# tensorflow/compression

Measured on AMD Instinct MI355X. Metric: Mpixels/s encode+decode round-trip (bit-exact), higher is better.
Workload: dtype int32

## Files before the change

compression_amd/csrc/range_pipe.h:

```cpp
#pragma once

#ifndef TFC_PIPE_TIMING
#define TFC_PIPE_TIMING 0
#endif

namespace tfc {

constexpr int kPipeTile = 256;
constexpr int kPipeEscMax = 32;
constexpr unsigned int kPipeBlock = 16;
constexpr unsigned int kPipeNoCall = 0x0001FFFFu;
constexpr unsigned int kPipeAggregate = 1u << 30;
constexpr unsigned int kPipePrefix = 2u << 30;
constexpr unsigned int kPipeRowsMask = (1u << 30) - 1u;

struct PipeEncArgs {
  const uint16_t* fast16;
  const int2* rows_fast;
  int ntab;
  int tab_entries;
  unsigned int* calls;
  unsigned int* status;
  unsigned int* done;
  unsigned int* fallback;
// ... 560 lines not shown
#endif
    while ((((v = sync[L::kSeq + b % L::kSlots]) & ~(L::kLast | L::kBail)) != b + 1u) && !(v & L::kBail)) __builtin_amdgcn_s_sleep(1);
    asm volatile("" ::: "memory");
#if TFC_PIPE_TIMING
    waited_words += clock64() - c0;
#endif
    return v;
  };

  unsigned int wa[kPipeBlock], wb[kPipeBlock];
  unsigned int seq = wait_words(0u);
  bool bail = (seq & L::kBail) != 0u;
  if (!bail) read_words(wa, 0u, 0u);
  unsigned int dig_done = 0u;
  for (unsigned int b = 0; !bail; ++b) {
    const bool last = (seq & L::kLast) != 0u;
    read_words(wb, b % L::kSlots, 1u);
    const unsigned int seq_early = last ? 0u : sync[L::kSeq + (b + 1u) % L::kSlots];
    if (dig_done + L::kDigSlots <= b) {
#if TFC_PIPE_TIMING
      const unsigned long long c0 = clock64();
#endif
      while ((dig_done = sync[L::kDigDone]) + L::kDigSlots <= b) __builtin_amdgcn_s_sleep(1);
#if TFC_PIPE_TIMING
      waited_digits += clock64() - c0;
#endif
    }
    const unsigned int dslot = b % L::kDigSlots;
    dstage = area + L::kDig + dslot * L::kDigSlot + L::kDigStride * lane;
    ds_off = area_off + L::kDig + dslot * L::kDigSlot + L::kDigStride * lane;
    n = 0u;
    block(wa);
    if (lane == 0u) sync[L::kConsumed] = b + 1u;
    if (!last) {
      seq = ((seq_early & ~(L::kLast | L::kBail)) == b + 2u || (seq_early & L::kBail)) ? seq_early : wait_words(b + 1u);
      if (seq & L::kBail) { bail = true; break; }
      read_words(wa, (b + 1u) % L::kSlots, 0u);
    }
    block(wb);
    reinterpret_cast<uint2*>(area + L::kRec)[dslot * 64u + lane] = make_uint2(wpos, n);
    overflow |= (n != 0u && wpos + ((n + 15u) & ~15u) > pa.cap) ? 1u : 0u;
    wpos += n;
    asm volatile("s_waitcnt lgkmcnt(0)" ::: "memory");
    if (lane == 0u) sync[L::kDigPub] = b + 1u;
    if (__any(too_long)) {
      bail = true;
      if (lane == 0u) atomicOr(&pa.fallback[job], 1u);
      break;
    }
    if (last) break;
  }
  asm volatile("s_waitcnt lgkmcnt(0)" ::: "memory");
  if (lane == 0u) sync[L::kExit] = 1u;
  if (gi == 0u && lane == 0u) {
    g_pipe_clock[0] = clock64() - clk0;
    g_pipe_clock[1] = wall_clock64() - wall0;
    g_pipe_clock[4] = waited_words;
    g_pipe_clock[6] = waited_digits;
#if TFC_PIPE_TIMING
    g_enc_clock[0] = t_blocks; g_enc_clock[1] = n_blocks; g_enc_clock[2] = n_redone; g_enc_clock[3] = t_redo;
#endif
  }
  if (bail) return;
  if (live) {
    pa.stage_state[static_cast<size_t>(gi) * 64 + lane] = make_uint4(base, s1, (hd & 0xFFFFu) | (had << 31), rn);
    pa.stage_out[static_cast<size_t>(gi) * 64 + lane] = make_uint2(wpos, overflow);
  }
}

__global__ void __launch_bounds__(64) enc_chain_direct_kernel(const PipeChainJobs jobs, const PipeEncArgs pa) {
  constexpr unsigned int kRows = PipeEncChainLds::kRows;
  constexpr unsigned int kDigits = 2 * kRows;
  constexpr int kStride = lane_stride(kDigits + 8);
  __shared__ __attribute__((aligned(16))) unsigned char stage[64 * kStride];
  const unsigned int gi = blockIdx.x;
  const unsigned int job = gi / static_cast<unsigned int>(pa.groups_per_job);
  const unsigned int gidx = gi % static_cast<unsigned int>(pa.groups_per_job);
  if (__hip_atomic_load(&pa.fallback[job], __ATOMIC_RELAXED, __HIP_MEMORY_SCOPE_AGENT) != 0u) return;
  const PipeChainJob& J = jobs.job[job];
  const unsigned int lane = threadIdx.x;
  const int64_t s = static_cast<int64_t>(gidx) * 64 + lane;
  const bool live = s < jobs.streams;

  uint4 st = live ? J.state[s] : make_uint4(0u, 0xFFFFFFFFu, 0u, 0u);
  unsigned int base = st.x, s1 = st.y, hd = st.z & 0xFFFFu, had = st.z >> 31, rn = st.w;
  lanes_pin(base, s1, hd, rn);

  const unsigned int ds_off = static_cast<unsigned int>(reinterpret_cast<size_t>(
                                  (__attribute__((address_space(3))) unsigned char*)stage)) + kStride * lane;
  unsigned char* const dstage = stage + kStride * lane;
  unsigned char* const out = J.chunk + (live ? s : 0) * static_cast<int64_t>(pa.cap);
  unsigned int wpos = 0u, n = 0u, overflow = 0u;

  auto put = [&](unsigned int d, bool on) {
    *reinterpret_cast<unsigned short*>(dstage + n) = __builtin_bswap16(static_cast<unsigned short>(d));
    n += on ? 2u : 0u;
  };
  auto flush = [&]() {
#pragma unroll
    for (unsigned int c = 0; c < kDigits / 16u; ++c) {
      if (16u * c < n) {
        uint2 v[2];
        v[0] = reinterpret_cast<const uint2*>(dstage)[2 * c];
        v[1] = reinterpret_cast<const uint2*>(dstage)[2 * c + 1];
        if (wpos + 16u * c + 16u <= pa.cap) lanes_gstore16(out + wpos + 16u * c, v[0], v[1]);
        else overflow = 1u;
      }
    }
    wpos += n;
    n = 0u;
  };
  auto put_run = [&](unsigned int fill, unsigned int bytes) {
    flush();
    for (unsigned int k = 0; k < bytes; k += 2u) {
      const unsigned short be = static_cast<unsigned short>(fill);
      if (wpos + 2u <= pa.cap) lanes_gstore_elem(reinterpret_cast<unsigned short*>(out + wpos), be);
      else overflow = 1u;
      wpos += 2u;
    }
  };
  auto call = [&](unsigned int lo, unsigned int hi, bool act) __attribute__((always_inline)) {
    const unsigned int a = scale16(s1, lo);
    const unsigned int b = scale16(s1, hi) - 1u;
    const unsigned int bs = base + a;
    const unsigned int t1 = b - a;
    const bool carry = act && bs < a;
    const bool ren = act && (t1 >> 16) == 0u;
    const unsigned int e = bs >> 16;
    const bool solid = ren && e != 0xFFFFu;
    const bool ffff = ren && e == 0xFFFFu;
    const bool held = had != 0u;
    const unsigned int X = (hd + (carry ? 1u : 0u)) & 0xFFFFu;
    const bool emit = held && (solid || (carry && (!ffff || rn != 0u)));
    put(X, emit);
    const unsigned int run_out = !held ? 0u : solid ? rn : (carry && rn != 0u) ? (ffff ? rn - 1u : rn) : 0u;
    if (__any(run_out != 0u)) {
      if (run_out != 0u) put_run(carry ? 0u : 0xFFFFu, 2u * run_out);
    }
    if (solid) {
      hd = e; had = 1u; rn = 0u;
    } else if (ffff) {
      if (!held) { hd = 0xFFFFu; had = 1u; rn = 0u; }
      else if (!carry) { rn += 1u; }
      else if (rn == 0u) { hd = X; rn = 1u; }
      else { hd = 0u; rn = 1u; }
    } else if (carry && held) {
      had = 0u; rn = 0u;
    }
    base = act ? (ren ? bs << 16 : bs) : base;
    s1 = act ? (ren ? (t1 << 16) | 0xFFFFu : t1) : s1;
  };

  const unsigned int nt = static_cast<unsigned int>(pa.nt);
  const unsigned int* const status = pa.status + static_cast<size_t>(gi) * nt * 64 + lane;
  const unsigned int* const done = pa.done + static_cast<size_t>(gi) * nt;
  unsigned int avail = 0u;
  unsigned int tn = 0u;
  bool bail = false;
  auto ensure = [&](unsigned int need) {
    while (tn < nt && __any(live && avail < need)) {
      const unsigned int* const flag = done + tn;
      long long t0 = 0;
      bool timing = false;
      while (__hip_atomic_load(flag, __ATOMIC_RELAXED, __HIP_MEMORY_SCOPE_AGENT) == 0u) {
        const long long now = static_cast<long long>(wall_clock64());
        if (!timing) { t0 = now; timing = true; }
        else if (now - t0 > pa.poll_ticks) { bail = true; return; }
        __builtin_amdgcn_s_sleep(8);
      }
      __builtin_amdgcn_fence(__ATOMIC_ACQUIRE, "agent");
      avail = __hip_atomic_load(status + static_cast<size_t>(tn) * 64, __ATOMIC_RELAXED, __HIP_MEMORY_SCOPE_AGENT) & kPipeRowsMask;
      ++tn;
      if (__hip_atomic_load(&pa.fallback[job], __ATOMIC_RELAXED, __HIP_MEMORY_SCOPE_AGENT) != 0u) { bail = true; return; }
    }
  };

  const unsigned char* const mine = reinterpret_cast<const unsigned char*>(pa.calls + static_cast<size_t>(gi) * 64 * pa.rows) + 128u * lane;
  unsigned int w[kRows] = {}, wn[kRows] = {};
  auto load_rows = [&](unsigned int b) {
    const unsigned char* p = mine + static_cast<size_t>(b) * (64u * kRows * 4u);
#pragma unroll
    for (unsigned int c = 0; c < kRows / 4u; ++c) {
      const uint4 v = lanes_gload16(p + 16u * c);
      wn[4 * c] = v.x; wn[4 * c + 1] = v.y; wn[4 * c + 2] = v.z; wn[4 * c + 3] = v.w;
    }
  };
  auto block = [&](unsigned int w0, unsigned int w1, unsigned int w2, unsigned int w3, unsigned int w4, unsigned int w5,
                   unsigned int w6, unsigned int w7, unsigned int w8, unsigned int w9, unsigned int w10, unsigned int w11,
                   unsigned int w12, unsigned int w13, unsigned int w14, unsigned int w15) __attribute__((always_inline)) {
    const unsigned int base0 = base, s10 = s1, hd0 = hd, had0 = had;
    unsigned int flag = rn, na = ds_off + n;
    asm volatile(
        "s_mov_b64 s[56:57], exec\n\t"
        "v_mov_b32 v101, 0\n\tv_mov_b32 v103, 0\n\t"
        TFC_PENC_STEP(W0) TFC_PENC_STEP(W1) TFC_PENC_STEP(W2) TFC_PENC_STEP(W3)
        TFC_PENC_STEP(W4) TFC_PENC_STEP(W5) TFC_PENC_STEP(W6) TFC_PENC_STEP(W7)
        TFC_PENC_STEP(W8) TFC_PENC_STEP(W9) TFC_PENC_STEP(W10) TFC_PENC_STEP(W11)
        TFC_PENC_STEP(W12) TFC_PENC_STEP(W13) TFC_PENC_STEP(W14) TFC_PENC_STEP(W15)
        "s_mov_b64 exec, s[56:57]\n\t"
        "s_waitcnt lgkmcnt(0)\n\t"
        : [BASE] "+v"(base), [S] "+v"(s1), [H] "+v"(hd), [HAD] "+v"(had), [NA] "+v"(na), [FLAG] "+v"(flag)
        : [NOCALL] "s"(kPipeNoCall), [K64K] "s"(0x10000u), [KFFFF] "s"(0xFFFFu), [KHI16] "s"(0xFFFF0000u), [PERM] "s"(0x0c0c0001u),
          [W0] "v"(w0), [W1] "v"(w1), [W2] "v"(w2), [W3] "v"(w3), [W4] "v"(w4), [W5] "v"(w5),
          [W6] "v"(w6), [W7] "v"(w7), [W8] "v"(w8), [W9] "v"(w9), [W10] "v"(w10), [W11] "v"(w11),
          [W12] "v"(w12), [W13] "v"(w13), [W14] "v"(w14), [W15] "v"(w15)
        : "vcc", "memory", "s52", "s53", "s56", "s57", "v100", "v101", "v102", "v103", "v104", "v105", "v106", "v107",
          "v108", "v109", "v110", "v111", "v112", "v113", "v114", "v115", "v117", "v118", "v119");
    if (__builtin_expect(!__any(flag != 0u), 1)) {
      n = na - ds_off;
    } else {
      base = base0; s1 = s10; hd = hd0; had = had0;
      const unsigned int ww[kPipeBlock] = {w0, w1, w2, w3, w4, w5, w6, w7, w8, w9, w10, w11, w12, w13, w14, w15};
#pragma nounroll
      for (unsigned int k = 0; k < kPipeBlock; ++k) {
        unsigned int word = ww[0];
#pragma unroll
        for (unsigned int q = 1; q < kPipeBlock; ++q) word = k == q ? ww[q] : word;
        const unsigned int hi = word >> 16;
        call(word & 0xFFFFu, hi == 0u ? 65536u : hi, word != kPipeNoCall);
      }
    }
  };

  ensure(kRows);
  if (!bail) load_rows(0u);
#pragma unroll
  for (unsigned int k = 0; k < kRows; ++k) asm volatile("" : "+v"(wn[k]));
  for (unsigned int b = 0; !bail && (tn < nt || __any(b * kRows < avail)); ++b) {
#pragma unroll
    for (unsigned int k = 0; k < kRows; ++k) w[k] = wn[k];
    ensure((b + 2u) * kRows);
    if (bail) break;
    load_rows(b + 1u);
    flush();
    if (__any(avail < (b + 1u) * kRows)) {
#pragma unroll
      for (unsigned int k = 0; k < kRows; ++k) w[k] = b * kRows + k < avail ? w[k] : kPipeNoCall;
    }
    block(w[0], w[1], w[2], w[3], w[4], w[5], w[6], w[7], w[8], w[9], w[10], w[11], w[12], w[13], w[14], w[15]);
    block(w[16], w[17], w[18], w[19], w[20], w[21], w[22], w[23], w[24], w[25], w[26], w[27], w[28], w[29], w[30], w[31]);
  }
  flush();
  if (bail) {
    if (lane == 0) atomicOr(&pa.fallback[job], 1u);
    return;
  }
  if (live) {
    pa.stage_state[static_cast<size_t>(gi) * 64 + lane] = make_uint4(base, s1, (hd & 0xFFFFu) | (had << 31), rn);
    pa.stage_out[static_cast<size_t>(gi) * 64 + lane] = make_uint2(wpos, overflow);
  }
}


__global__ void enc_gate_kernel(const unsigned int* started, unsigned int want, long long ticks) {
  const long long t0 = static_cast<long long>(wall_clock64());
  while (__hip_atomic_load(started, __ATOMIC_RELAXED, __HIP_MEMORY_SCOPE_AGENT) < want &&
         static_cast<long long>(wall_clock64()) - t0 < ticks)
    __builtin_amdgcn_s_sleep(8);
}

__global__ void __launch_bounds__(64) enc_commit_kernel(const PipeChainJobs jobs, const PipeEncArgs pa) {
  const unsigned int gi = blockIdx.x;
  const unsigned int job = gi / static_cast<unsigned int>(pa.groups_per_job);
  const unsigned int gidx = gi % static_cast<unsigned int>(pa.groups_per_job);
  if (pa.fallback[job] != 0u) return;
  const int64_t s = static_cast<int64_t>(gidx) * 64 + threadIdx.x;
  if (s >= jobs.streams) return;
  const PipeChainJob& J = jobs.job[job];
  J.state[s] = pa.stage_state[static_cast<size_t>(gi) * 64 + threadIdx.x];
  const uint2 o = pa.stage_out[static_cast<size_t>(gi) * 64 + threadIdx.x];
  J.chunk_len[s] = o.y ? 0u : o.x;
  if (o.y) atomicOr(J.overflow_flag, 1u);
}


constexpr unsigned int kPipeSkipRow = 0xFFFFu;
__device__ inline unsigned int pipe_raw_entry(unsigned int sym_or_bit, int M) { return (M != 0 ? 0x8000u : 0u) | sym_or_bit; }
__device__ inline int pipe_mode_step(int M, unsigned int bit) {
  if (M < 0) return bit ? -M : (M == -31 ? 32 : M - 1);
  return M - 1;
}

struct PipeDecArgs {
  unsigned short* raw;
  unsigned int* posrec;
  unsigned int* kend;
  uint4* state_out;
  const unsigned short* rowaddr;
  unsigned int* fallback;
  unsigned int* progress;
  unsigned int* tile_done;
  unsigned int* started;
  int rows;
  int groups_per_job;
  int groups;
  int concurrent;
  long long poll_ticks;
};
constexpr unsigned int kPipeFinal = 0x80000000u;
#ifndef TFC_PIPE_RELEASE
#define TFC_PIPE_RELEASE 64
#endif
constexpr unsigned int kPipeRelease = TFC_PIPE_RELEASE;
struct PipeDecJob { const uint8_t* blob; const long long* off; const uint4* state; };
struct PipeDecJobs {
  int64_t streams, elems;
  int blocks_per_job, n;
  PipeDecJob job[64];
};

struct PipeRowJobs {
  int64_t per_job;
  int ntab, n;
  struct { const int32_t* index; unsigned long long* first_error; } job[64];
};
__global__ void __launch_bounds__(256) dec_rows_kernel(const PipeRowJobs jobs, unsigned short* rowaddr) {
  const int k = blockIdx.y;
  const int32_t* index = jobs.job[k].index;
  unsigned short* out = rowaddr + static_cast<size_t>(k) * jobs.per_job;
  for (int64_t i = static_cast<int64_t>(blockIdx.x) * 1024 + threadIdx.x, e = min(jobs.per_job, (static_cast<int64_t>(blockIdx.x) + 1) * 1024);
       i < e; i += 256) {
    int t = tfc_gload(index + i);
    if (t < 0 || t >= jobs.ntab) {
      atomicMin(jobs.job[k].first_error, static_cast<unsigned long long>(i));
      t = 0;
    }
    out[i] = static_cast<unsigned short>(16 * t);
  }
}

struct PipeDecLds {
  static constexpr int kWords = 2 * kPipeBlock * 2 / 8 + 4;
  static constexpr int kStride = lane_stride(8 * kWords);
  static constexpr int kCodes = 0;
  static constexpr int kRows = kCodes + 64 * kStride;
  static constexpr int kBytes = kRows + 64 * kStride;
  static constexpr int kStage = kPipeBlock * 128;
};

#ifndef TFC_PDEC_ABL
#define TFC_PDEC_ABL 0
#endif
#if TFC_PDEC_ABL & 1
#define TFC_PDEC_STORE(KOFF)
#define TFC_PDEC_WAIT2 "s_waitcnt lgkmcnt(1)\n\t"
#else
#define TFC_PDEC_STORE(KOFF) "ds_write_b16 %[STG], v117 offset:" #KOFF "\n\t"
#define TFC_PDEC_WAIT2 "s_waitcnt lgkmcnt(2)\n\t"
#endif
#ifndef TFC_PDEC_PAD
#define TFC_PDEC_PAD 0
#endif
#define TFC_PDEC_PAD2 "v_mov_b32 v139, v139\n\tv_mov_b32 v139, v139\n\t"
#if TFC_PDEC_PAD == 1
#define TFC_PDEC_PAD_A TFC_PDEC_PAD2
#elif TFC_PDEC_PAD == 5
#define TFC_PDEC_PAD_A "s_waitcnt lgkmcnt(15)\n\ts_waitcnt lgkmcnt(15)\n\t"
#else
#define TFC_PDEC_PAD_A
#endif
#if TFC_PDEC_PAD == 2
#define TFC_PDEC_PAD_B TFC_PDEC_PAD2
#else
#define TFC_PDEC_PAD_B
#endif
#if TFC_PDEC_PAD == 3
#define TFC_PDEC_PAD_C TFC_PDEC_PAD2
#else
#define TFC_PDEC_PAD_C
#endif
#if TFC_PDEC_PAD == 4
#define TFC_PDEC_PAD_D TFC_PDEC_PAD2
#else
#define TFC_PDEC_PAD_D
#endif
#define TFC_PDEC_STEP(KOFF, MI, MO, AHEAD, NEXT, PWSTEP)                                    \
  "v_cvt_f32_u32 v111, %[S]\n\t"                                                          \
  "v_add_f32 v111, 1.0, v111\n\t"                                                         \
  "v_rcp_f32 v111, v111\n\t"                                                              \
  TFC_PDEC_PAD_A                                                                          \
  "v_cvt_f32_u32 v110, %[D]\n\t"                                                          \
  "v_fma_f32 v110, -v110, %[SCALE], -%[HSCALE]\n\t"                                       \
  "v_fma_f32 v110, v110, v111, -1.0\n\t"                                                  \
  "v_cvt_i32_f32 v110, v110\n\t"                                                          \
  "v_ashrrev_i32 v111, 6, v110\n\t"                                                       \
  "s_waitcnt lgkmcnt(0)\n\t"                                                              \
  "v_mad_i32_i24 v112, v111, -8, v106\n\t"                                                \
  "ds_read_b64 v[114:115], v112\n\t"                                                      \
  "v_mad_i32_i24 v113, v111, -2, v107\n\t"                                                \
  "ds_read_u16 v116, v113\n\t"                                                            \
  AHEAD                                                                                   \
  "v_cndmask_b32_e64 v133, 0, 2, s[56:57]\n\t"                                            \
  "v_add_u32 %[CP], %[CP], v133\n\t"                                                      \
  "ds_read_u16 v109, %[CP]\n\t"                                                           \
  "v_ashrrev_i32 v137, 31, " MI "\n\t"                                                    \
  "v_cmp_le_u32_sdwa vcc, v110, v105 src0_sel:WORD_0 src1_sel:WORD_1\n\t"                 \
  "v_cndmask_b32 v137, v136, v137, vcc\n\t"                                               \
  "v_xor_b32 " MO ", v135, v137\n\t"                                                      \
  "v_cmpx_le_u32 vcc, v130, v131\n\t"                                                     \
  TFC_PDEC_PAD_B                                                                          \
  "s_waitcnt lgkmcnt(1)\n\t"                                                              \
  "v_lshlrev_b64 v[118:119], v110, v[114:115]\n\t"                                        \
  "v_bcnt_u32_b32 v116, v118, v116\n\t"                                                   \
  "v_bcnt_u32_b32 v117, v119, v116\n\t"                                                   \
  "v_lshl_add_u32 v112, v117, 1, v104\n\t"                                                \
  "ds_read_u16_d16_hi v122, v112 offset:2\n\t"                                            \
  "ds_read_u16_d16_hi v124, v112 offset:4\n\t"                                            \
  TFC_PDEC_PAD_C                                                                          \
  TFC_PDEC_STORE(KOFF)                                                                    \
  "v_subrev_co_u32 v135, vcc, 1, " MO "\n\t"                                              \
  "v_cndmask_b32_e64 v136, 0, -1, vcc\n\t"                                                \
  "v_add_u32 v140, " #PWSTEP ", %[PW]\n\t"                                                \
  "v_cndmask_b32 %[PW], %[PW], v140, vcc\n\t"                                             \
  "v_cndmask_b32 v142, %[BINROW], " NEXT ", vcc\n\t"                                      \
  "ds_read_b128 v[104:107], v142\n\t"                                                     \
  TFC_PDEC_WAIT2                                                                          \
  TFC_PDEC_PAD_D                                                                          \
  "v_mad_u64_u32 v[126:127], s[52:53], v122, %[S], v[122:123]\n\t"                        \
  "v_mad_u64_u32 v[128:129], s[52:53], v124, %[S], v[124:125]\n\t"                        \
  "v_add_u32 v129, -1, v129\n\t"                                                          \
  "v_min_u32 v129, v129, %[S]\n\t"                                                        \
  "v_sub_u32 v131, v129, v127\n\t"                                                        \
  "v_cmp_gt_u32_e64 s[56:57], %[K64K], v131\n\t"                                          \
  "v_lshl_or_b32 v132, v131, 16, %[KFFFF]\n\t"                                            \
  "v_cndmask_b32_e64 %[S], v131, v132, s[56:57]\n\t"                                      \
  "v_sub_u32 v130, %[D], v127\n\t"                                                        \
  "v_perm_b32 v132, v130, v109, %[PERM]\n\t"                                              \
  "v_cndmask_b32_e64 %[D], v130, v132, s[56:57]\n\t"
#define TFC_PDEC_STEP_H(KOFF, MI, MO, AHEAD, NEXT, PWSTEP)                                  \
  "v_cvt_f32_u32 v111, %[S]\n\t"                                                          \
  "v_add_f32 v111, 1.0, v111\n\t"                                                         \
  "v_rcp_f32 v111, v111\n\t"                                                              \
  "v_cvt_f32_u32 v110, %[D]\n\t"                                                          \
  "v_fma_f32 v110, -v110, %[SCALE], -%[HSCALE]\n\t"                                       \
  "v_fma_f32 v110, v110, v111, -1.0\n\t"                                                  \
  "v_cvt_i32_f32 v110, v110\n\t"                                                          \
  "v_ashrrev_i32 v143, 1, v110\n\t"                                                       \
  "v_ashrrev_i32 v111, 6, v143\n\t"                                                       \
  "s_waitcnt lgkmcnt(0)\n\t"                                                              \
  "v_mad_i32_i24 v112, v111, -8, v106\n\t"                                                \
  "ds_read_b64 v[114:115], v112\n\t"                                                      \
  "v_mad_i32_i24 v113, v111, -2, v107\n\t"                                                \
  "ds_read_u16 v116, v113\n\t"                                                            \
  AHEAD                                                                                   \
  "v_cndmask_b32_e64 v133, 0, 2, s[56:57]\n\t"                                            \
  "v_add_u32 %[CP], %[CP], v133\n\t"                                                      \
  "ds_read_u16 v109, %[CP]\n\t"                                                           \
  "v_ashrrev_i32 v137, 31, " MI "\n\t"                                                    \
  "v_cmp_le_u32_sdwa vcc, v110, v105 src0_sel:WORD_0 src1_sel:WORD_1\n\t"                 \
  "v_cndmask_b32 v137, v136, v137, vcc\n\t"                                               \
  "v_xor_b32 " MO ", v135, v137\n\t"                                                      \
  "v_cmpx_le_u32 vcc, v130, v131\n\t"                                                     \
  "v_mad_i32_i24 v141, v110, %[NSH], %[NSH]\n\t"                                          \
  "s_waitcnt lgkmcnt(1)\n\t"                                                              \
  "v_lshlrev_b64 v[118:119], v143, v[114:115]\n\t"                                        \
  "v_bcnt_u32_b32 v116, v118, v116\n\t"                                                   \
  "v_bcnt_u32_b32 v117, v119, v116\n\t"                                                   \
  "v_lshl_add_u32 v112, v117, 2, v104\n\t"                                                \
  "ds_read2_b32 v[144:145], v112 offset1:1\n\t"                                           \
  "v_subrev_co_u32 v135, vcc, 1, " MO "\n\t"                                              \
  "v_cndmask_b32_e64 v136, 0, -1, vcc\n\t"                                                \
  "v_add_u32 v140, " #PWSTEP ", %[PW]\n\t"                                                \
  "v_cndmask_b32 %[PW], %[PW], v140, vcc\n\t"                                             \
  "v_cndmask_b32 v142, %[BINROW], " NEXT ", vcc\n\t"                                      \
  "ds_read_b128 v[104:107], v142\n\t"                                                     \
  "s_waitcnt lgkmcnt(1)\n\t"                                                              \
  "v_cmp_ge_u32_sdwa vcc, v141, v144 src0_sel:DWORD src1_sel:WORD_1\n\t"                  \
  "v_cndmask_b32_sdwa v122, v144, v144, vcc dst_sel:WORD_1 dst_unused:UNUSED_PAD src0_sel:WORD_0 src1_sel:WORD_1\n\t" \
  "v_cndmask_b32_sdwa v124, v144, v145, vcc dst_sel:WORD_1 dst_unused:UNUSED_PAD src0_sel:WORD_1 src1_sel:WORD_0\n\t" \
  "v_addc_co_u32_e64 v117, s[58:59], v117, v117, vcc\n\t"                                 \
  "v_cmp_ge_u32_sdwa vcc, v141, v145 src0_sel:DWORD src1_sel:WORD_0\n\t"                  \
  "v_cndmask_b32_sdwa v122, v122, v145, vcc dst_sel:WORD_1 dst_unused:UNUSED_PAD src0_sel:WORD_1 src1_sel:WORD_0\n\t" \
  "v_cndmask_b32_sdwa v124, v124, v145, vcc dst_sel:WORD_1 dst_unused:UNUSED_PAD src0_sel:WORD_1 src1_sel:WORD_1\n\t" \
  "v_addc_co_u32_e64 v117, s[58:59], v117, v123, vcc\n\t"                                 \
  TFC_PDEC_STORE(KOFF)                                                                    \
  "v_mad_u64_u32 v[126:127], s[52:53], v122, %[S], v[122:123]\n\t"                        \
  "v_mad_u64_u32 v[128:129], s[52:53], v124, %[S], v[124:125]\n\t"                        \
  "v_add_u32 v129, -1, v129\n\t"                                                          \
  "v_min_u32 v129, v129, %[S]\n\t"                                                        \
  "v_sub_u32 v131, v129, v127\n\t"                                                        \
  "v_cmp_gt_u32_e64 s[56:57], %[K64K], v131\n\t"                                          \
  "v_lshl_or_b32 v132, v131, 16, %[KFFFF]\n\t"                                            \
  "v_cndmask_b32_e64 %[S], v131, v132, s[56:57]\n\t"                                      \
  "v_sub_u32 v130, %[D], v127\n\t"                                                        \
  "v_perm_b32 v132, v130, v109, %[PERM]\n\t"                                              \
  "v_cndmask_b32_e64 %[D], v130, v132, s[56:57]\n\t"
#define TFC_PDEC_STEP_CH(KOFF, MI, MO) TFC_PDEC_STEP(KOFF, MI, MO, "", "v140", 16)
#define TFC_PDEC_STEP_IX(KOFF, MI, MO) TFC_PDEC_STEP(KOFF, MI, MO, "ds_read_u16 v108, %[PW] offset:2\n\t", "v108", 2)
#define TFC_PDEC_STEP_PCH(KOFF, MI, MO) TFC_PDEC_STEP_H(KOFF, MI, MO, "", "v140", 16)
#define TFC_PDEC_STEP_PIX(KOFF, MI, MO) TFC_PDEC_STEP_H(KOFF, MI, MO, "ds_read_u16 v108, %[PW] offset:2\n\t", "v108", 2)
#define TFC_PDEC_STEP2(STEP, K0, K1) STEP(K0, "%[M]", "v138") STEP(K1, "v138", "%[M]")
#define TFC_PDEC_BLOCK_HEAD                                                               \
  "v_mov_b32 v104, %[R0]\n\tv_mov_b32 v105, %[R1]\n\tv_mov_b32 v106, %[R2]\n\tv_mov_b32 v107, %[R3]\n\t" \
  "v_mov_b32 v122, 0\n\tv_mov_b32 v123, 0\n\tv_mov_b32 v124, 0\n\tv_mov_b32 v125, 0\n\t"       \
  "v_mov_b32 v130, 0\n\tv_mov_b32 v131, 0\n\ts_mov_b64 s[56:57], 0\n\t"                   \
  "v_subrev_co_u32 v135, vcc, 1, %[M]\n\tv_cndmask_b32_e64 v136, 0, -1, vcc\n\t"           \
  "s_mov_b64 s[54:55], exec\n\tv_mov_b32 %[FLAG], 1\n\t"
#define TFC_PDEC_BLOCK_TAIL                                                               \
  "v_cndmask_b32_e64 v133, 0, 2, s[56:57]\n\t"                                            \
  "v_add_u32 %[CP], %[CP], v133\n\t"                                                      \
  "s_waitcnt lgkmcnt(0)\n\t"                                                              \
  "v_cmpx_le_u32 vcc, v130, v131\n\tv_mov_b32 %[FLAG], 0\n\ts_mov_b64 exec, s[54:55]\n\t"   \
  "v_mov_b32 %[R0], v104\n\tv_mov_b32 %[R1], v105\n\tv_mov_b32 %[R2], v106\n\tv_mov_b32 %[R3], v107\n\t"
#define TFC_PDEC_ONE(STEP) TFC_PDEC_BLOCK_HEAD STEP(0, "%[M]", "v138") "v_mov_b32 %[M], v138\n\t" TFC_PDEC_BLOCK_TAIL
#define TFC_PDEC_BLOCK(STEP)                                                              \
  TFC_PDEC_BLOCK_HEAD                                                                     \
  TFC_PDEC_STEP2(STEP, 0, 128) TFC_PDEC_STEP2(STEP, 256, 384) TFC_PDEC_STEP2(STEP, 512, 640)            \
  TFC_PDEC_STEP2(STEP, 768, 896) TFC_PDEC_STEP2(STEP, 1024, 1152) TFC_PDEC_STEP2(STEP, 1280, 1408)      \
  TFC_PDEC_STEP2(STEP, 1536, 1664) TFC_PDEC_STEP2(STEP, 1792, 1920)                       \
  TFC_PDEC_BLOCK_TAIL

template <bool INDEXED, bool PAIRS>
__global__ void __launch_bounds__(512) dec_chain_kernel(const PipeDecJobs jobs, const LaneArgs la, const PipeDecArgs pa) {
  extern __shared__ unsigned char lanes_lds[];
  lanes_load_image(lanes_lds, la);
  using L = PipeDecLds;
  if constexpr (!PAIRS) {
    const unsigned int entries = static_cast<unsigned int>(la.ntab) + kDirRepeat + 1u;
    const unsigned int nw = max(1u, (1u << la.precision) >> 6) + 1u;
    for (unsigned int i = threadIdx.x; i < entries; i += blockDim.x) {
      if (i >= static_cast<unsigned int>(la.ntab) && i + 1u != entries) continue;
      const LaneRow* e = reinterpret_cast<const LaneRow*>(lanes_lds) + i;
      *reinterpret_cast<unsigned long long*>(lanes_lds + e->bits) &= ~1ull;
      *reinterpret_cast<unsigned short*>(lanes_lds + e->cum) = 0;
    }
    __syncthreads();
    {
      const LaneRow* e = reinterpret_cast<const LaneRow*>(lanes_lds) + (entries - 1u);
      for (unsigned int w = threadIdx.x; w < nw; w += blockDim.x)
        *reinterpret_cast<unsigned short*>(lanes_lds + e->cum + 2u * w) += 0x8000u;
    }
    __syncthreads();
    for (unsigned int i = threadIdx.x; i < entries; i += blockDim.x) {
      LaneRow* e = reinterpret_cast<LaneRow*>(lanes_lds) + i;
      const unsigned int info = e->info, limit = info & 0x7FFFu, esc = info >> 31;
      unsigned int esclo = 0xFFFFu;
      if (i + 1u == entries) esclo = 1u << (la.precision - 1);
      else if (esc) esclo = lds_u16(lanes_lds, e->cdf + 2u * limit + 2u) >> (16 - la.precision);
      e->info = limit | (esc << 15) | ((0xFFFFu - esclo) << 16);
      e->bits -= 8u;
      e->cum -= 2u;
      if (i + 1u == entries) e->cdf -= 0x10000u;
    }
    __syncthreads();
  }

  const unsigned long long clk0 = clock64(), wall0 = wall_clock64();
  if (threadIdx.x == 0u) __hip_atomic_fetch_add(pa.started, 1u, __ATOMIC_RELAXED, __HIP_MEMORY_SCOPE_AGENT);
  const unsigned int job = blockIdx.x / static_cast<unsigned int>(jobs.blocks_per_job);
  const unsigned int wv = (blockIdx.x % static_cast<unsigned int>(jobs.blocks_per_job)) * (blockDim.x >> 6) + (threadIdx.x >> 6);
  if (wv >= static_cast<unsigned int>(pa.groups_per_job)) return;
  const unsigned int gi = job * static_cast<unsigned int>(pa.groups_per_job) + wv;
  const PipeDecJob& J = jobs.job[job];
  const unsigned int lane = threadIdx.x & 63u;
  const int64_t s = static_cast<int64_t>(wv) * 64 + lane;
  const bool live = s < jobs.streams;
  const unsigned int elems = live ? static_cast<unsigned int>(jobs.elems) : 0u;

  const uint4 st = live ? J.state[s] : make_uint4(0u, 0xFFFFFFFFu, 0u, 2u);
  unsigned int D = st.z - st.x;
  unsigned int s1 = st.y;
  const long long o0 = live ? J.off[s] : 0;
  unsigned int len = live ? static_cast<unsigned int>(J.off[s + 1] - o0) : 0u;
  unsigned int pos_start = 2u * st.w;
  lanes_pin(D, s1, len, pos_start);

  const unsigned int lds0 = static_cast<unsigned int>(reinterpret_cast<size_t>(
      (__attribute__((address_space(3))) unsigned char*)lanes_lds));
  const unsigned int wave_off = static_cast<unsigned int>(la.lds_image) + (threadIdx.x >> 6) * static_cast<unsigned int>(la.lds_wave);
  LaneWindow<L::kWords> cw;
  const unsigned int cw_off = wave_off + L::kCodes + L::kStride * lane;
  cw.lds = lanes_lds + cw_off;
  cw.g = J.blob + o0;
  cw.len = len;
  cw.request(pos_start);
  cw.base = pos_start;
  unsigned int cp = cw_off;
  LaneWindow<L::kWords> iw;
  const unsigned int iw_off = wave_off + L::kRows + L::kStride * lane;
  if (INDEXED) {
    iw.lds = lanes_lds + iw_off;
    iw.g = reinterpret_cast<const unsigned char*>(pa.rowaddr + (static_cast<size_t>(job) * jobs.streams + (live ? s : 0)) * jobs.elems);
    iw.len = elems * 2u;
    iw.request(0u);
    iw.base = 0u;
  }

  const unsigned int stg_off = wave_off + (INDEXED ? L::kBytes : L::kRows);
  const unsigned int stg = stg_off + 2u * lane;
  bool staged = false;
  unsigned int staged_k = 0u;

  const float scale = static_cast<float>(1u << la.precision);
  float hscale = scale;
  asm volatile("" : "+v"(hscale));
  const unsigned int cp_max = (1u << la.precision) - 1u;
  const unsigned int pair_sh = 16u - static_cast<unsigned int>(la.precision);
  const unsigned int pair_nsh = 0u - (1u << pair_sh);
  const unsigned int dir_end = 16u * static_cast<unsigned int>(la.ntab);
  const unsigned int bin_addr = dir_end + 16u * kDirRepeat;
  uint4 bin = *reinterpret_cast<const uint4*>(lanes_lds + bin_addr);
  asm volatile("" : "+v"(bin.x), "+v"(bin.y), "+v"(bin.z), "+v"(bin.w));
  unsigned int bin_addr_v = bin_addr;
  asm volatile("" : "+v"(bin_addr_v));

  unsigned int pos = 0u;
  int M = 0;
  unsigned int pw = INDEXED ? iw_off : 0u;
  uint4 R = make_uint4(0u, 0u, 0u, 0u);
  bool row_loaded = false;

  unsigned short* const raw = pa.raw + static_cast<size_t>(gi) * pa.rows * 64;
  unsigned int* const posrec = pa.posrec + static_cast<size_t>(gi) * (pa.rows / kPipeBlock + 1) * 64 + lane;
  unsigned int k = 0u;
  auto flush = [&]() {
    if (!staged) return;
#if TFC_PDEC_ABL & 4
    staged = false;
    return;
#endif
    unsigned char* dst = reinterpret_cast<unsigned char*>(raw + static_cast<size_t>(staged_k) * 64) + 16u * lane;
#pragma unroll
    for (unsigned int j = 0; j < L::kStage / 1024u; ++j) {
      const uint4 v = *reinterpret_cast<const uint4*>(lanes_lds + stg_off + 1024u * j + 16u * lane);
      lanes_gstore16(dst + 1024u * j, make_uint2(v.x, v.y), make_uint2(v.z, v.w));
    }
    staged = false;
  };

  auto load_row = [&]() {
    const unsigned int a = INDEXED ? static_cast<unsigned int>(*reinterpret_cast<const unsigned short*>(lanes_lds + pw)) : pw;
    R = *reinterpret_cast<const uint4*>(lanes_lds + a);
  };

  auto gstep = [&](bool act, unsigned int row, bool to_stage = false) {
    unsigned int entry = 0u;
    if (act) {
      const unsigned int dig = __builtin_bswap16(*reinterpret_cast<const unsigned short*>(lanes_lds + cp));
      if (M == 0) {
        const float fq = (static_cast<float>(D) + 0.5f) * __builtin_amdgcn_rcpf(static_cast<float>(s1)) * scale;
        const unsigned int q = min(static_cast<unsigned int>(fq), cp_max);
        if constexpr (PAIRS) {
          const unsigned int j = q >> 1, w = j >> 6;
          const unsigned long long word = *reinterpret_cast<const unsigned long long*>(lanes_lds + R.z + 8u + 8u * w);
          const unsigned int cum = *reinterpret_cast<const unsigned short*>(lanes_lds + R.w + 2u + 2u * w);
          const unsigned long long below = ~0ull >> (63u - (j & 63u));
          const unsigned int i = cum + static_cast<unsigned int>(__popcll(word & below));
          const unsigned int Q = q << pair_sh;
          unsigned int u = 2u * i;
          u += Q >= lds_u16(lanes_lds, R.x + 2u * u + 2u) ? 1u : 0u;
          u += (u & 1u) != 0u && Q >= lds_u16(lanes_lds, R.x + 4u * i + 4u) ? 1u : 0u;
          unsigned int lo = lds_u16(lanes_lds, R.x + 2u * u), hi = lds_u16(lanes_lds, R.x + 2u * u + 2u);
          unsigned int A = scale16(s1, lo);
          unsigned int b = scale16(s1, hi) - 1u;
          b = hi == 0u ? s1 : b;
          for (int fix = 0; fix < 4; ++fix) {
            if (D - A > b - A) {
              if (D < A) u = u > 0u ? u - 1u : 0u;
              else if (hi != 0u) u = u + 1u;
              lo = lds_u16(lanes_lds, R.x + 2u * u);
              hi = lds_u16(lanes_lds, R.x + 2u * u + 2u);
              A = scale16(s1, lo);
              b = scale16(s1, hi) - 1u;
              b = hi == 0u ? s1 : b;
            }
          }
          D -= A;
          s1 = b - A;
          const bool ren = (s1 >> 16) == 0u;
          D = ren ? (D << 16) | dig : D;
          s1 = ren ? (s1 << 16) | 0xFFFFu : s1;
          cp += ren ? 2u : 0u;
          entry = u;
          M = ((R.y >> 15) & 1u) != 0u && lo == ((0xFFFFu - (R.y >> 16)) << pair_sh) ? -1 : 0;
        } else {
        const unsigned int w = q >> 6;
        const unsigned long long word = *reinterpret_cast<const unsigned long long*>(lanes_lds + R.z + 8u + 8u * w);
        const unsigned int cum = *reinterpret_cast<const unsigned short*>(lanes_lds + R.w + 2u + 2u * w);
        const unsigned long long below = ~0ull >> (63u - (q & 63u));
        unsigned int sym = cum + static_cast<unsigned int>(__popcll(word & below));
        unsigned int lo = lds_u16(lanes_lds, R.x + 2u * sym + 2u);
        unsigned int hi = lds_u16(lanes_lds, R.x + 2u * sym + 4u);
        unsigned int A = scale16(s1, lo);
        unsigned int b = scale16(s1, hi) - 1u;
        b = hi == 0u ? s1 : b;
        const unsigned int nsym = (R.y & 0x7FFFu) + ((R.y >> 15) & 1u);
        for (int fix = 0; fix < 4; ++fix) {
          if (D - A > b - A) {
            if (D < A) sym = sym > 0u ? sym - 1u : 0u;
            else sym = sym + 1u < nsym ? sym + 1u : nsym - 1u;
            lo = lds_u16(lanes_lds, R.x + 2u * sym + 2u);
            hi = lds_u16(lanes_lds, R.x + 2u * sym + 4u);
            A = scale16(s1, lo);
            b = scale16(s1, hi) - 1u;
            b = hi == 0u ? s1 : b;
          }
        }
        D -= A;
        s1 = b - A;
        const bool ren = (s1 >> 16) == 0u;
        D = ren ? (D << 16) | dig : D;
        s1 = ren ? (s1 << 16) | 0xFFFFu : s1;
        cp += ren ? 2u : 0u;
        entry = pipe_raw_entry(sym, 0);
        M = ((R.y >> 15) & 1u) != 0u && sym == (R.y & 0x7FFFu) ? -1 : 0;
        }
      } else {
        const unsigned int half = scale16(s1, 32768u);
        const unsigned int bit = D >= half ? 1u : 0u;
        const unsigned int A = bit ? half : 0u;
        const unsigned int b = bit ? s1 : half - 1u;
        D -= A;
        s1 = b - A;
        const bool ren = (s1 >> 16) == 0u;
        D = ren ? (D << 16) | dig : D;
        s1 = ren ? (s1 << 16) | 0xFFFFu : s1;
        cp += ren ? 2u : 0u;
        entry = PAIRS ? 0x8001u + bit : pipe_raw_entry(bit, M);
        if (M < 0) {
          if (bit) M = -M;
          else M = M == -31 ? 32 : M - 1;
        } else {
          --M;
        }
      }
      if (M == 0) {
        ++pos;
        pw += INDEXED ? 2u : 16u;
        if (!INDEXED && pw == dir_end) pw = 0u;
        load_row();
      } else {
        R = bin;
      }
      if (to_stage) *reinterpret_cast<unsigned short*>(lanes_lds + stg + 128u * (row - k)) = static_cast<unsigned short>(entry);
      else raw[static_cast<size_t>(row) * 64 + lane] = static_cast<unsigned short>(entry);
    }
  };

#if TFC_PIPE_TIMING
  unsigned long long t_asm = 0ull, n_asm = 0ull, t_commit = 0ull, t_rest = 0ull;
#endif
  static_assert(8 * L::kWords >= 4 * kPipeBlock + 2, "a window holds two blocks and the entry read ahead");
  constexpr unsigned int kWindowNeed = 4u * kPipeBlock + 2u;
  struct WindowRefill {
    uint2 code[L::kWords], rows[L::kWords];
    unsigned int code_pos, rows_pos;
    bool code_pending, rows_pending;
  };
  unsigned int n_phase = 0u, n_refill = 0u, n_irefill = 0u;
  auto park = [&](const WindowRefill& rq) __attribute__((always_inline)) {
#if TFC_PIPE_TIMING
    const unsigned long long tm0 = clock64();
#endif
    if (rq.code_pending) {
      const unsigned int cpos = cw.base + (cp - cw_off);
      cw.commit(rq.code_pos, rq.code);
      cp = cw_off + (cpos - cw.base);
    }
    if (INDEXED && rq.rows_pending) {
      iw.commit(rq.rows_pos, rq.rows);
      pw = iw_off + (2u * pos - iw.base);
    }
#if TFC_PIPE_TIMING
    asm volatile("s_waitcnt lgkmcnt(0)" ::: "memory");
    t_commit += clock64() - tm0;
#endif
  };
  auto phase_decide = [&](WindowRefill& rq) __attribute__((always_inline)) {
#if TFC_PIPE_TIMING
    const unsigned long long tm1 = clock64();
#endif
    flush();
    if (k != 0u && (k / kPipeBlock) % kPipeRelease == 0u) {
      posrec[static_cast<size_t>(k / kPipeBlock) * 64] = pos + (M != 0 ? 1u : 0u);
      __builtin_amdgcn_fence(__ATOMIC_RELEASE, "agent");
      if (lane == 0u) __hip_atomic_store(&pa.progress[gi], k, __ATOMIC_RELAXED, __HIP_MEMORY_SCOPE_AGENT);
    }
    posrec[static_cast<size_t>(k / kPipeBlock) * 64] = pos + (M != 0 ? 1u : 0u);
    ++n_phase;
    rq.code_pos = cw.base + (cp - cw_off);
    rq.code_pending = !__all((cp - cw_off) + kWindowNeed <= 8u * L::kWords);
    rq.rows_pos = 2u * pos;
    rq.rows_pending = INDEXED && !__all((rq.rows_pos - iw.base) + kWindowNeed <= 8u * L::kWords);
    n_refill += rq.code_pending ? 1u : 0u;
    n_irefill += rq.rows_pending ? 1u : 0u;
#if TFC_PIPE_TIMING
    t_rest += clock64() - tm1;
#endif
  };
  auto phase_request = [&](WindowRefill& rq) __attribute__((always_inline)) {
#if TFC_PIPE_TIMING
    const unsigned long long tm1 = clock64();
#endif
    if (rq.code_pending) {
      cw.request(rq.code_pos, rq.code);
    } else {
#pragma unroll
      for (int w = 0; w < L::kWords; ++w) asm("" : "=v"(rq.code[w].x), "=v"(rq.code[w].y));
    }
    if (INDEXED) {
      if (rq.rows_pending) {
        iw.request(rq.rows_pos, rq.rows);
      } else {
#pragma unroll
        for (int w = 0; w < L::kWords; ++w) asm("" : "=v"(rq.rows[w].x), "=v"(rq.rows[w].y));
      }
    }
#if TFC_PIPE_TIMING
    t_rest += clock64() - tm1;
#endif
  };
  auto memory_phase = [&](WindowRefill& rq) __attribute__((always_inline)) {
    phase_decide(rq);
    phase_request(rq);
  };
  auto fast_block = [&](unsigned int& flag) __attribute__((always_inline)) {
#define TFC_PDEC_OPERANDS                                                                                              \
        : [D] "+v"(D), [S] "+v"(s1), [CP] "+v"(cp), [M] "+v"(M), [PW] "+v"(pw), [FLAG] "+v"(flag),                    \
          [R0] "+v"(R.x), [R1] "+v"(R.y), [R2] "+v"(R.z), [R3] "+v"(R.w)                                              \
        : [STG] "v"(stg), [BINROW] "v"(bin_addr_v), [SCALE] "s"(scale), [HSCALE] "v"(hscale),        \
          [K64K] "s"(0x10000u), [KFFFF] "s"(0xFFFFu), [PERM] "s"(0x05040001u), [NSH] "s"(pair_nsh) \
        : "vcc", "memory", "s52", "s53", "s54", "s55", "s56", "s57", "s58", "s59", "v104", "v105", "v106", "v107", "v108", "v109", "v110", "v111", "v112", "v113", \
          "v114", "v115", "v116", "v117", "v118", "v119", "v122", "v123", "v124", "v125", "v126", "v127", "v128",      \
          "v129", "v130", "v131", "v132", "v133", "v134", "v135", "v136", "v137", "v138", "v139", "v140", "v141", "v142", "v143", "v144", "v145"
#if TFC_PIPE_TIMING
    const unsigned long long ta = clock64();
#endif
    if constexpr (INDEXED && PAIRS) asm volatile(TFC_PDEC_BLOCK(TFC_PDEC_STEP_PIX) TFC_PDEC_OPERANDS);
    else if constexpr (PAIRS) asm volatile(TFC_PDEC_BLOCK(TFC_PDEC_STEP_PCH) TFC_PDEC_OPERANDS);
    else if constexpr (INDEXED) asm volatile(TFC_PDEC_BLOCK(TFC_PDEC_STEP_IX) TFC_PDEC_OPERANDS);
    else asm volatile(TFC_PDEC_BLOCK(TFC_PDEC_STEP_CH) TFC_PDEC_OPERANDS);
#if TFC_PIPE_TIMING
    t_asm += clock64() - ta;
    ++n_asm;
#endif
  };
  auto fast_step = [&](unsigned int& flag, unsigned int slot) __attribute__((always_inline)) {
    const unsigned int stg_row = stg + 128u * slot;
    {
      const unsigned int stg = stg_row;
      if constexpr (INDEXED && PAIRS) asm volatile(TFC_PDEC_ONE(TFC_PDEC_STEP_PIX) TFC_PDEC_OPERANDS);
      else if constexpr (PAIRS) asm volatile(TFC_PDEC_ONE(TFC_PDEC_STEP_PCH) TFC_PDEC_OPERANDS);
      else if constexpr (INDEXED) asm volatile(TFC_PDEC_ONE(TFC_PDEC_STEP_IX) TFC_PDEC_OPERANDS);
      else asm volatile(TFC_PDEC_ONE(TFC_PDEC_STEP_CH) TFC_PDEC_OPERANDS);
    }
#undef TFC_PDEC_OPERANDS
  };
  cw.commit();
  if (INDEXED) iw.commit();
  bool gave_up = false;
  while (__any(pos < elems)) {
    if (lds0 == 0u && row_loaded && (INDEXED || static_cast<unsigned int>(la.ntab) >= kPipeBlock)) {
      while (__all(!live || (pos + kPipeBlock <= elems && M > -16)) && k + kPipeBlock <= static_cast<unsigned int>(pa.rows)) {
        WindowRefill rq;
        phase_decide(rq);
        auto block = [&]() __attribute__((always_inline)) {
          const unsigned int D0 = D, s10 = s1, cp0 = cp, pw0 = pw;
          const int M0 = M;
          const uint4 R0 = R;
          unsigned int flag = 0u;
          fast_block(flag);
          if (__builtin_expect(__any(live && flag != 0u), 0)) {
            D = D0; s1 = s10; cp = cp0; pw = pw0; M = M0; R = R0;
  #pragma nounroll
            for (unsigned int i = 0; i < kPipeBlock; ++i) {
              const unsigned int D1 = D, s11 = s1, cp1 = cp, pw1 = pw;
              const int M1 = M;
              const uint4 R1 = R;
              unsigned int f1 = 0u;
              if (live) fast_step(f1, i);
              if (__any(live && f1 != 0u)) {
                D = D1; s1 = s11; cp = cp1; pw = pw1; M = M1; R = R1;
                gstep(live, k + i, true);
              } else {
                pos += (pw - pw1) / (INDEXED ? 2u : 16u);
                if (!INDEXED) pw -= pw >= dir_end ? dir_end : 0u;
              }
            }
          } else {
            pos += (pw - pw0) / (INDEXED ? 2u : 16u);
            if (!INDEXED) pw -= pw >= dir_end ? dir_end : 0u;
          }
          staged = true;
          staged_k = k;
          k += kPipeBlock;
        };
        if (rq.code_pending || rq.rows_pending) {
          phase_request(rq);
          block();
          park(rq);
        } else {
          block();
        }
      }
      if (!__any(pos < elems)) break;
    }
    if (k + kPipeBlock > static_cast<unsigned int>(pa.rows)) {
      gave_up = true;
      break;
    }
    WindowRefill rq;
    memory_phase(rq);
    if (!row_loaded) {
      if (M == 0) load_row(); else R = bin;
      row_loaded = true;
    }
    const bool whole = pos + kPipeBlock <= elems;
    const bool blocks = __any(whole);
    if (blocks && __any(!whole && pos < elems && M != 0)) {
      if (pos < elems) {
#pragma unroll
        for (unsigned int i = 0; i < kPipeBlock; ++i) raw[static_cast<size_t>(k + i) * 64 + lane] = static_cast<unsigned short>(kPipeSkipRow);
      }
#pragma nounroll
      for (unsigned int i = 0; i < kPipeBlock; ++i) gstep(!whole && pos < elems && M != 0, k + i);
      k += kPipeBlock;
      park(rq);
      continue;
    }
    const bool busy = blocks ? whole : pos < elems;
    const bool sitting = blocks && !whole && pos < elems;
    if (__builtin_expect(lds0 == 0u && blocks && !__any(busy && M <= -16), 1)) {
      if (__any(sitting)) {
        if (sitting) {
#pragma unroll
          for (unsigned int i = 0; i < kPipeBlock; ++i) *reinterpret_cast<unsigned short*>(lanes_lds + stg + 128u * i) = static_cast<unsigned short>(kPipeSkipRow);
        }
      }
      const unsigned int D0 = D, s10 = s1, cp0 = cp, pw0 = pw;
      const int M0 = M;
      const uint4 R0 = R;
      unsigned int flag = 0u;
      if (busy) {
        fast_block(flag);
      }
      if (__builtin_expect(!__any(flag != 0u), 1)) {
        if (busy) {
          pos += (pw - pw0) / (INDEXED ? 2u : 16u);
        }
        if (!INDEXED)
          while (__any(busy && pw >= dir_end)) pw -= pw >= dir_end ? dir_end : 0u;
        staged = true;
        staged_k = k;
        k += kPipeBlock;
        park(rq);
        continue;
      }
      D = D0; s1 = s10; cp = cp0; pw = pw0; M = M0; R = R0;
    }
    if (sitting) {
#pragma unroll
      for (unsigned int i = 0; i < kPipeBlock; ++i) raw[static_cast<size_t>(k + i) * 64 + lane] = static_cast<unsigned short>(kPipeSkipRow);
    }
#pragma nounroll
    for (unsigned int i = 0; i < kPipeBlock; ++i) gstep(busy && pos < elems, k + i);
    k += kPipeBlock;
    park(rq);
  }
  flush();
  posrec[static_cast<size_t>(k / kPipeBlock) * 64] = pos;
  if (gave_up) {
    if (lane == 0) {
      atomicOr(&pa.fallback[job], 1u);
      __hip_atomic_store(&pa.progress[gi], kPipeFinal, __ATOMIC_RELEASE, __HIP_MEMORY_SCOPE_AGENT);
    }
    return;
  }
  if (lane == 0) pa.kend[gi] = k;
  __builtin_amdgcn_fence(__ATOMIC_RELEASE, "agent");
  if (lane == 0) __hip_atomic_store(&pa.progress[gi], k | kPipeFinal, __ATOMIC_RELAXED, __HIP_MEMORY_SCOPE_AGENT);
  if (gi == 0 && lane == 0) {
    g_pipe_clock[2] = clock64() - clk0;
    g_pipe_clock[3] = wall_clock64() - wall0;
    g_pipe_window[0] = n_phase;
    g_pipe_window[1] = n_refill;
    g_pipe_window[2] = n_irefill;
#if TFC_PIPE_TIMING
    g_pipe_clock[5] = t_asm | (t_commit << 32);
    g_pipe_clock[7] = n_asm | (static_cast<unsigned long long>(k) << 16) | (t_rest << 32);
#endif
  }
  if (live) {
    const unsigned int cpos = cw.base + (cp - cw_off);
    const unsigned char* srcp = J.blob + o0;
    unsigned int window = 0u;
    for (int i = -4; i < 0; ++i) {
      const long long q = static_cast<long long>(cpos) + i;
      window = (window << 8) | ((q >= 0 && q < static_cast<long long>(len)) ? srcp[q] : 0u);
    }
    pa.state_out[static_cast<size_t>(gi) * 64 + lane] = make_uint4(window - D, s1, window, cpos >> 1);
  }
}

constexpr int kParseRows = 128;
constexpr unsigned int kParseMargin = 96;

constexpr int kParseEscTables = 2048;

struct PipePairMap { const int* adjust; };
template <bool INDEXED, bool PAIRS, typename Dst>
__global__ void __launch_bounds__(256) dec_parse_kernel(const DecLaneJobs<Dst> jobs, const PipeDecArgs pa, const DecRow* dir, int ntab,
                                                        const PipePairMap pm) {
  constexpr int kPitch = 66;
  __shared__ unsigned short buf[kParseRows * kPitch];
  __shared__ unsigned int escsym[kParseEscTables];
  __shared__ unsigned int incomplete;
  const unsigned int tiles = static_cast<unsigned int>(pa.rows) / kParseRows + 1u;
  const unsigned int gi = blockIdx.x % static_cast<unsigned int>(pa.groups), kt = blockIdx.x / static_cast<unsigned int>(pa.groups);
  const unsigned int job = gi / static_cast<unsigned int>(pa.groups_per_job);
  const unsigned int wv = gi % static_cast<unsigned int>(pa.groups_per_job);
  const DecLaneJob<Dst>& J = jobs.job[job];
  const unsigned int tid = threadIdx.x, lane = tid & 63u;
  const unsigned int k0 = kt * kParseRows;
  unsigned int* const tile_done = pa.tile_done + static_cast<size_t>(gi) * tiles + kt;
  unsigned int kend;
  bool final = true;
  if (pa.concurrent) {
    const unsigned int need = k0 + kParseRows + kParseMargin;
    unsigned int* const abandon = pa.started + 1;
    unsigned int v = 0u;
    if (tid == 0u) {
      unsigned int seen = ~0u, go = 1u;
      long long t0 = 0;
      if (__hip_atomic_load(abandon, __ATOMIC_RELAXED, __HIP_MEMORY_SCOPE_AGENT) != 0u) go = 0u;
      while (go) {
        v = __hip_atomic_load(&pa.progress[gi], __ATOMIC_RELAXED, __HIP_MEMORY_SCOPE_AGENT);
        if ((v & kPipeFinal) || v >= need) break;
        const long long now = static_cast<long long>(wall_clock64());
        if (v != seen) { seen = v; t0 = now; }
        else if (now - t0 > pa.poll_ticks) {
          __hip_atomic_store(abandon, 1u, __ATOMIC_RELAXED, __HIP_MEMORY_SCOPE_AGENT);
          go = 0u;
          break;
        }
        __builtin_amdgcn_s_sleep(32);
      }
      incomplete = go ? v : 0xFFFFFFFFu;
    }
    __syncthreads();
    v = incomplete;
    __syncthreads();
    if (v == 0xFFFFFFFFu) return;
    __builtin_amdgcn_fence(__ATOMIC_ACQUIRE, "agent");
    if (__hip_atomic_load(&pa.fallback[job], __ATOMIC_RELAXED, __HIP_MEMORY_SCOPE_AGENT) != 0u) return;
    final = (v & kPipeFinal) != 0u;
    kend = v & ~kPipeFinal;
    if (tid == 0u) incomplete = 0u;
  } else {
    if (pa.fallback[job] != 0u) return;
    if (kt == 0u && tid < 64u) {
      const int64_t s = static_cast<int64_t>(wv) * 64 + tid;
      if (s < jobs.streams) J.state[s] = pa.state_out[static_cast<size_t>(gi) * 64 + tid];
    }
    if (*tile_done != 0u) return;
    kend = pa.kend[gi];
  }
  if (k0 >= kend) return;
  const unsigned short* const raw = pa.raw + static_cast<size_t>(gi) * pa.rows * 64;
  const unsigned int nrows = min(static_cast<unsigned int>(kParseRows), kend - k0);
  for (unsigned int r = tid >> 6; r < nrows; r += 4u) buf[r * kPitch + lane] = raw[static_cast<size_t>(k0 + r) * 64 + lane];
  const bool esc_lds = ntab <= kParseEscTables;
  if (esc_lds)
    for (int i = tid; i < ntab; i += 256) {
      escsym[i] = (static_cast<unsigned int>(dir[i].w) & 0xFFFFu) | (PAIRS ? static_cast<unsigned int>(pm.adjust[i] + 2) << 16 : 0u);
    }
  __syncthreads();
  const unsigned int bitshift = PAIRS ? 1u : 0u;
  const unsigned int* const posrec = pa.posrec + static_cast<size_t>(gi) * (pa.rows / kPipeBlock + 1) * 64;
  const Dst dst = J.dst;
  const unsigned long long lt = (1ull << lane) - 1ull;
  const unsigned int untab = static_cast<unsigned int>(ntab);
  auto walk = [&](auto in_lds) __attribute__((always_inline)) {
  constexpr bool esc_in_lds = decltype(in_lds)::value;
  for (unsigned int l = tid >> 6; l < 64u; l += 4u) {
    const int64_t s = static_cast<int64_t>(wv) * 64 + l;
    if (s >= jobs.streams) continue;
    unsigned int p = posrec[static_cast<size_t>(k0 / kPipeBlock) * 64 + l];
    const unsigned int p1 = posrec[static_cast<size_t>((k0 + nrows) / kPipeBlock) * 64 + l];
    const int64_t base = s * jobs.elems;
    unsigned int pmod = p % untab;
    for (unsigned int c = 0; c < nrows; c += 64u) {
      const unsigned int i = c + lane;
      const unsigned int e = i < nrows ? buf[i * kPitch + l] : kPipeSkipRow;
      const bool start = (e & 0x8000u) == 0u;
      const unsigned long long mask = __ballot(start);
      const unsigned int before = static_cast<unsigned int>(__popcll(mask & lt));
      const unsigned int ord = p + before;
      const unsigned int total = static_cast<unsigned int>(__popcll(mask));
      if (start && ord < p1) {
        const int64_t at = base + ord;
        int t;
        if (INDEXED) {
          t = tfc_gload(J.index + at);
          t = (t < 0 || t >= ntab) ? 0 : t;
        } else {
          unsigned int m = pmod + before;
          if (untab >= 64u) m -= m >= untab ? untab : 0u;
          else m %= untab;
          t = static_cast<int>(m);
        }
        int v = static_cast<int>(e);
        const unsigned int ew = esc_in_lds ? escsym[t] : 0u;
        if constexpr (PAIRS) v += esc_in_lds ? static_cast<int>(ew >> 16) - 2 : pm.adjust[t];
        const int es = esc_in_lds ? static_cast<int>(static_cast<short>(ew & 0xFFFFu)) : dir[t].w;
        if (v == es) {
          unsigned int val = 0u;
          bool neg = false, closed = false;
          int m = -1;
          for (unsigned int q = k0 + i + 1u; q < kend; ++q) {
            const unsigned int x = q - k0 < nrows ? buf[(q - k0) * kPitch + l]
                                                  : *reinterpret_cast<const TFC_AS1 unsigned short*>((const TFC_AS1 void*)(raw + static_cast<size_t>(q) * 64 + l));
            const unsigned int bit = (x >> bitshift) & 1u;
            if (x == kPipeSkipRow) continue;
            if (m < 0) {
              if (bit) val = 1u << (-m - 1);
              else if (m == -31) val = 1u << 31;
            } else if (m > 1) {
              val |= bit << (m - 2);
            } else {
              neg = bit != 0u;
              closed = true;
              break;
            }
            m = pipe_mode_step(m, bit);
          }
          if (!closed && !final) incomplete = 1u;
          v = neg ? -static_cast<int>(val) : static_cast<int>(val) + es - 1;
        }
        dst.store(at, t, v);
      }
      p += total;
      pmod = (pmod + total) % untab;
    }
  }
  };
  if (esc_lds) walk(std::true_type{}); else walk(std::false_type{});
  if (pa.concurrent) {
    __syncthreads();
    if (tid == 0u && incomplete == 0u) *tile_done = 1u;
  }
}

}
```

Before: 64580.

## Prefetch staged decode rows into registers and write position records only at tile edges

```diff
diff --git a/compression_amd/csrc/range_pipe.h b/compression_amd/csrc/range_pipe.h
--- a/compression_amd/csrc/range_pipe.h
+++ b/compression_amd/csrc/range_pipe.h
@@ -886,6 +886,10 @@
 #define TFC_PIPE_RELEASE 64
 #endif
 constexpr unsigned int kPipeRelease = TFC_PIPE_RELEASE;
+constexpr int kParseRows = 128;
+constexpr unsigned int kPipeRecordEvery = kParseRows / kPipeBlock;
+static_assert(kParseRows % kPipeBlock == 0, "a parse tile is whole blocks: its edges have block records");
+static_assert((kPipeRelease * kPipeBlock) % kParseRows == 0, "a release ends on a tile edge: its own block's record is written");
 struct PipeDecJob { const uint8_t* blob; const long long* off; const uint4* state; };
 struct PipeDecJobs {
   int64_t streams, elems;
@@ -1211,6 +1215,27 @@
     }
     staged = false;
   };
+  struct StagedRows { uint4 v[L::kStage / 1024u]; };
+  auto read_staged = [&](StagedRows& sv) __attribute__((always_inline)) {
+#pragma unroll
+    for (unsigned int j = 0; j < L::kStage / 1024u; ++j) {
+#if TFC_PDEC_ABL & 4
+      asm("" : "=v"(sv.v[j].x), "=v"(sv.v[j].y), "=v"(sv.v[j].z), "=v"(sv.v[j].w));
+#else
+      sv.v[j] = *reinterpret_cast<const uint4*>(lanes_lds + stg_off + 1024u * j + 16u * lane);
+#endif
+    }
+  };
+  auto flush_read = [&](const StagedRows& sv) __attribute__((always_inline)) {
+    if (!staged) return;
+#if !(TFC_PDEC_ABL & 4)
+    unsigned char* dst = reinterpret_cast<unsigned char*>(raw + static_cast<size_t>(k - kPipeBlock) * 64) + 16u * lane;
+#pragma unroll
+    for (unsigned int j = 0; j < L::kStage / 1024u; ++j)
+      lanes_gstore16(dst + 1024u * j, make_uint2(sv.v[j].x, sv.v[j].y), make_uint2(sv.v[j].z, sv.v[j].w));
+#endif
+    staged = false;
+  };
 
   auto load_row = [&]() {
     const unsigned int a = INDEXED ? static_cast<unsigned int>(*reinterpret_cast<const unsigned short*>(lanes_lds + pw)) : pw;
@@ -1350,17 +1375,20 @@
     t_commit += clock64() - tm0;
 #endif
   };
-  auto phase_decide = [&](WindowRefill& rq) __attribute__((always_inline)) {
+  auto phase_decide = [&](WindowRefill& rq, auto flush_rows) __attribute__((always_inline)) {
 #if TFC_PIPE_TIMING
     const unsigned long long tm1 = clock64();
 #endif
-    flush();
-    if (k != 0u && (k / kPipeBlock) % kPipeRelease == 0u) {
+    flush_rows();
+    if ((k / kPipeBlock) % kPipeRecordEvery == 0u) {
+#if !(TFC_PDEC_ABL & 8)
       posrec[static_cast<size_t>(k / kPipeBlock) * 64] = pos + (M != 0 ? 1u : 0u);
-      __builtin_amdgcn_fence(__ATOMIC_RELEASE, "agent");
-      if (lane == 0u) __hip_atomic_store(&pa.progress[gi], k, __ATOMIC_RELAXED, __HIP_MEMORY_SCOPE_AGENT);
-    }
-    posrec[static_cast<size_t>(k / kPipeBlock) * 64] = pos + (M != 0 ? 1u : 0u);
+#endif
+      if (k != 0u && (k / kPipeBlock) % kPipeRelease == 0u) {
+        __builtin_amdgcn_fence(__ATOMIC_RELEASE, "agent");
+        if (lane == 0u) __hip_atomic_store(&pa.progress[gi], k, __ATOMIC_RELAXED, __HIP_MEMORY_SCOPE_AGENT);
+      }
+    }
     ++n_phase;
     rq.code_pos = cw.base + (cp - cw_off);
     rq.code_pending = !__all((cp - cw_off) + kWindowNeed <= 8u * L::kWords);
@@ -1395,7 +1423,7 @@
 #endif
   };
   auto memory_phase = [&](WindowRefill& rq) __attribute__((always_inline)) {
-    phase_decide(rq);
+    phase_decide(rq, flush);
     phase_request(rq);
   };
   auto fast_block = [&](unsigned int& flag) __attribute__((always_inline)) {
@@ -1435,15 +1463,20 @@
   bool gave_up = false;
   while (__any(pos < elems)) {
     if (lds0 == 0u && row_loaded && (INDEXED || static_cast<unsigned int>(la.ntab) >= kPipeBlock)) {
+      flush();
+      StagedRows sv;
+#pragma unroll
+      for (unsigned int j = 0; j < L::kStage / 1024u; ++j) asm("" : "=v"(sv.v[j].x), "=v"(sv.v[j].y), "=v"(sv.v[j].z), "=v"(sv.v[j].w));
       while (__all(!live || (pos + kPipeBlock <= elems && M > -16)) && k + kPipeBlock <= static_cast<unsigned int>(pa.rows)) {
         WindowRefill rq;
-        phase_decide(rq);
+        phase_decide(rq, [&]() __attribute__((always_inline)) { flush_read(sv); });
         auto block = [&]() __attribute__((always_inline)) {
           const unsigned int D0 = D, s10 = s1, cp0 = cp, pw0 = pw;
           const int M0 = M;
           const uint4 R0 = R;
           unsigned int flag = 0u;
           fast_block(flag);
+          read_staged(sv);
           if (__builtin_expect(__any(live && flag != 0u), 0)) {
             D = D0; s1 = s10; cp = cp0; pw = pw0; M = M0; R = R0;
   #pragma nounroll
@@ -1461,6 +1494,7 @@
                 if (!INDEXED) pw -= pw >= dir_end ? dir_end : 0u;
               }
             }
+            read_staged(sv);
           } else {
             pos += (pw - pw0) / (INDEXED ? 2u : 16u);
             if (!INDEXED) pw -= pw >= dir_end ? dir_end : 0u;
@@ -1576,7 +1610,6 @@
   }
 }
 
-constexpr int kParseRows = 128;
 constexpr unsigned int kParseMargin = 96;
 
 constexpr int kParseEscTables = 2048;
```

Result: faster. 65900, median of 6 (+2.0%).
